# RoyiAvital/QuadraticProgramSolver

Measured on AMD Instinct MI355X. Metric: ADMM iterations/sec, higher is better.
Workload: dtype f64

## Files before the change

### quadraticprogramsolver_amd/csrc/k_loop.hip

```cpp
#include <cstdlib>

#include "qps_kernels.h"
#include "wave_reduce.h"
#include <hip/hip_ext.h>

namespace qps {

namespace {

template <typename T> __device__ __forceinline__ T wave_sum(T v) { return wave_sum_all(v); }
__device__ __forceinline__ unsigned long long absbits(double v) { return (unsigned long long)__double_as_longlong(fabs(v)); }
__device__ __forceinline__ unsigned long long wave_max_u64(unsigned long long v) {
#pragma unroll
    for (int o = 32; o > 0; o >>= 1) { unsigned long long t = __shfl_xor(v, o, 64); v = t > v ? t : v; }
    return v;
}

template <typename T, int RB, int TRI, int THREADS>
__global__ __launch_bounds__(THREADS) void k_gemv_rows(const T* __restrict__ S, int64_t ld, const T* __restrict__ v,
                                                   T* __restrict__ out, const T* __restrict__ out0, T alpha, T beta,
                                                   int r0, int c0, int c1, BatchStride bs) {
    using V = typename VecOf<T>::type;
    if (bs.active && !bs.active[blockIdx.y]) return;
    S += (int64_t)blockIdx.y * bs.mat; v += (int64_t)blockIdx.y * bs.vin; out += (int64_t)blockIdx.y * bs.vout;
// ... 30 lines not shown
            }
        }
    }
    __shared__ T red[THREADS / 64][RB];
#pragma unroll
    for (int i = 0; i < RB; ++i) acc[i] = wave_sum(acc[i]);
    if ((tid & 63) == 0) {
#pragma unroll
        for (int i = 0; i < RB; ++i) red[tid >> 6][i] = acc[i];
    }
    __syncthreads();
    if (tid < RB) {
        T s = T(0);
#pragma unroll
        for (int w = 0; w < THREADS / 64; ++w) s += red[w][tid];
        T r = alpha * s;
        if (beta != T(0)) r += beta * out0[rb + tid];
        out[rb + tid] = r;
    }
}

constexpr int GC_RT = 32;
template <typename T>
__global__ __launch_bounds__(256) void k_gemv_cols(const T* __restrict__ S, int64_t ld, const T* __restrict__ va,
                                                   const T* __restrict__ vb, T ca, T cb, T* __restrict__ part,
                                                   int64_t part_ld, int ncols) {
    using V = typename VecOf<T>::type;
    constexpr int VN = VecOf<T>::N;
    const int c = (blockIdx.x * 256 + threadIdx.x) * VN;
    if (c >= ncols) return;
    const int rt = blockIdx.y;
    const int rbase = rt * GC_RT;
    T acc[VN];
#pragma unroll
    for (int e = 0; e < VN; ++e) acc[e] = T(0);
    const T* Sp = S + (int64_t)rbase * ld + c;
#pragma unroll 8
    for (int i = 0; i < GC_RT; ++i) {
        T w = ca * va[rbase + i];
        if (vb) w += cb * vb[rbase + i];
        typedef T NV __attribute__((ext_vector_type(VN)));
        const NV a = __builtin_nontemporal_load(reinterpret_cast<const NV*>(Sp + (int64_t)i * ld));
#pragma unroll
        for (int e = 0; e < VN; ++e) acc[e] += a[e] * w;
    }
    V o;
    T* op = reinterpret_cast<T*>(&o);
#pragma unroll
    for (int e = 0; e < VN; ++e) op[e] = acc[e];
    *reinterpret_cast<V*>(part + (int64_t)rt * part_ld + c) = o;
}

template <typename T>
__global__ __launch_bounds__(256) void k_colsum(const T* __restrict__ part, int64_t part_ld, int ntiles,
                                                const T* __restrict__ a0, T s0, const T* __restrict__ a1, T s1,
                                                T* __restrict__ out, int ncols, BatchStride bs) {
    using V = typename VecOf<T>::type;
    constexpr int VN = VecOf<T>::N;
    if (bs.active && !bs.active[blockIdx.y]) return;
    part += (int64_t)blockIdx.y * bs.mat; out += (int64_t)blockIdx.y * bs.vout;
    if (a0) a0 += (int64_t)blockIdx.y * bs.vin;
    if (a1) a1 += (int64_t)blockIdx.y * bs.vin;
    constexpr int COLS = 128 / (int)sizeof(T);
    constexpr int CL = COLS / VN;
    constexpr int TL = 256 / CL;
    const int cl = threadIdx.x % CL, tl = threadIdx.x / CL;
    const int c = blockIdx.x * COLS + cl * VN;
    T acc[VN];
#pragma unroll
    for (int e = 0; e < VN; ++e) acc[e] = T(0);
    if (c < ncols) {
        int t = tl;
        for (; t + 7 * TL < ntiles; t += 8 * TL) {
            V v[8];
#pragma unroll
            for (int j = 0; j < 8; ++j) v[j] = *reinterpret_cast<const V*>(part + (int64_t)(t + TL * j) * part_ld + c);
#pragma unroll
            for (int j = 0; j < 8; ++j) {
                const T* vp = reinterpret_cast<const T*>(&v[j]);
#pragma unroll
                for (int e = 0; e < VN; ++e) acc[e] += vp[e];
            }
        }
        for (; t < ntiles; t += TL) {
            const V v = *reinterpret_cast<const V*>(part + (int64_t)t * part_ld + c);
            const T* vp = reinterpret_cast<const T*>(&v);
#pragma unroll
            for (int e = 0; e < VN; ++e) acc[e] += vp[e];
        }
    }
    __shared__ T red[TL][COLS + 1];
#pragma unroll
    for (int e = 0; e < VN; ++e) red[tl][cl * VN + e] = acc[e];
    __syncthreads();
    constexpr int PL = 256 / COLS;
    static_assert(TL % PL == 0 && (PL == 16 || PL == 8), "slab lanes per output");
    const int o = threadIdx.x / PL, pl = threadIdx.x % PL;
    T s = T(0);
#pragma unroll
    for (int k = 0; k < TL / PL; ++k) s += red[pl * (TL / PL) + k][o];
    s = (PL == 16) ? row16_sum_last(s) : oct_sum_all(s);
    const int oc = blockIdx.x * COLS + o;
    if (pl == PL - 1 && oc < ncols) {
        T r = s;
        if (a0) r += s0 * a0[oc];
        if (a1) r += s1 * a1[oc];
        out[oc] = r;
    }
}

template <typename T>
__global__ __launch_bounds__(256) void k_admm_update(int NP, int MP, const T* __restrict__ xx, const T* __restrict__ zz,
                                                     T* __restrict__ x, T* __restrict__ xp, T* __restrict__ z,
                                                     T* __restrict__ zp, T* __restrict__ y, const T* __restrict__ l,
                                                     const T* __restrict__ u, T alpha, T rho) {
    const int i = blockIdx.x * 256 + threadIdx.x;
    const T alpha1 = T(1) - alpha, rho1 = T(1) / rho;
    if (i < NP) {
        const T xo = x[i];
        xp[i] = xo;
        x[i] = alpha * xx[i] + alpha1 * xo;
    }
    if (i < MP) {
        const T zo = z[i], yo = y[i], zt = zz[i];
        zp[i] = zo;
        T t = alpha * zt + alpha1 * zo + rho1 * yo;
        const T lo = l[i], hi = u[i];
        const T zn = t > hi ? hi : (t < lo ? lo : t);
        z[i] = zn;
        y[i] = yo + rho * (alpha * zt + alpha1 * zo - zn);
    }
}

template <typename T>
__global__ __launch_bounds__(256) void k_check_norms(int n, int m, const T* __restrict__ Ax, const T* __restrict__ Px,
                                                     const T* __restrict__ Aty, const T* __restrict__ q,
                                                     const T* __restrict__ x, const T* __restrict__ xp,
                                                     const T* __restrict__ z, const T* __restrict__ zp,
                                                     unsigned long long* __restrict__ slots, int dual_only, BatchStride bs) {
    if (bs.active && !bs.active[blockIdx.y]) return;
    {
        const int64_t on = (int64_t)blockIdx.y * bs.vin, om = (int64_t)blockIdx.y * bs.vout;
        Ax += om; z += om; zp += om; Px += on; Aty += on; q += on; x += on; xp += on; slots += (int64_t)blockIdx.y * 16;
    }
    unsigned long long v[9];
#pragma unroll
    for (int k = 0; k < 9; ++k) v[k] = 0ull;
    for (int i = blockIdx.x * 256 + threadIdx.x; i < max(n, m); i += gridDim.x * 256) {
        if (i < m && !dual_only) {
            const double ax = (double)Ax[i], zi = (double)z[i];
            v[0] = max(v[0], absbits((double)(Ax[i] - z[i])));
            v[2] = max(v[2], absbits(ax));
            v[3] = max(v[3], absbits(zi));
            v[8] = max(v[8], absbits((double)(z[i] - zp[i])));
        }
        if (i < n) {
            v[1] = max(v[1], absbits((double)(Px[i] + q[i] + Aty[i])));
            v[4] = max(v[4], absbits((double)Px[i]));
            v[5] = max(v[5], absbits((double)Aty[i]));
            v[6] = max(v[6], absbits((double)q[i]));
            if (!dual_only) v[7] = max(v[7], absbits((double)(x[i] - xp[i])));
        }
    }
#pragma unroll
    for (int k = 0; k < 9; ++k) {
        v[k] = wave_max_u64(v[k]);
        if ((threadIdx.x & 63) == 0 && v[k] != 0ull) atomicMax(&slots[k], v[k]);
    }
}

__device__ __forceinline__ double jmax(double a, double b) { return (isnan(a) || isnan(b)) ? (double)NAN : (a > b ? a : b); }

__global__ void k_check_decide(const unsigned long long* __restrict__ slots, double* __restrict__ res, CheckScalars cs,
                               const double* __restrict__ rho_arr, const double* __restrict__ rhorho_arr,
                               const int* __restrict__ active) {
    if (threadIdx.x != 0) return;
    const int b = blockIdx.x;
    if (active && !active[b]) return;
    slots += (int64_t)b * 16; res += (int64_t)b * 8;
    if (rho_arr) { cs.rho = rho_arr[b]; cs.rhorho = rhorho_arr[b]; cs.convFlag = 1; }
    double nv[9];
    for (int k = 0; k < 9; ++k) nv[k] = __longlong_as_double((long long)slots[k]);
    const double MIN_VAL_RHO = 1e-3, MAX_VAL_RHO = 1e6;
    const double normResPrim = nv[0], normResDual = nv[1];
    const double maxNormPrim = jmax(nv[2], nv[3]);
    const double maxNormDual = jmax(jmax(nv[4], nv[5]), nv[6]);
    double rhorho = cs.rhorho;
    if (cs.adptRho) {
        const double numeratorVal = normResPrim * maxNormDual;
        const double denominatorVal = normResDual * maxNormPrim;
        const double t = cs.rho * sqrt(numeratorVal / denominatorVal);
        rhorho = t > MAX_VAL_RHO ? MAX_VAL_RHO : (t < MIN_VAL_RHO ? MIN_VAL_RHO : t);
    }
    const double epsPrim = cs.epsAbs + cs.epsRel * maxNormPrim;
    const double epsDual = cs.epsAbs + cs.epsRel * maxNormDual;
    int flag = cs.convFlag;
    if ((normResPrim < epsPrim) && (normResDual < epsDual)) flag = 3;
    if ((nv[7] <= cs.epsAdmm) && (nv[8] <= cs.epsAdmm)) flag = 2;
    res[0] = normResPrim; res[1] = normResDual; res[2] = maxNormPrim; res[3] = maxNormDual;
    res[4] = rhorho; res[5] = (double)flag; res[6] = nv[7]; res[7] = nv[8];
}

template <typename T> __global__ void k_fill(T* p, int64_t n, T v) {
    int64_t i = (int64_t)blockIdx.x * 256 + threadIdx.x;
    if (i < n) p[i] = v;
}
template <typename T> __global__ void k_convert(const double* __restrict__ s, T* __restrict__ d, int64_t n) {
    int64_t i = (int64_t)blockIdx.x * 256 + threadIdx.x;
    if (i < n) d[i] = (T)s[i];
}
template <typename T> __global__ void k_convert_back(const T* __restrict__ s, double* __restrict__ d, int64_t n) {
    int64_t i = (int64_t)blockIdx.x * 256 + threadIdx.x;
    if (i < n) d[i] = (double)s[i];
}

}

static int env_int(const char* name, int dflt) { const char* e = getenv(name); return e ? atoi(e) : dflt; }

template <typename T, int RB, int TH>
static void gemv_rows_launch(hipStream_t st, const T* S, int64_t ld, const T* v, T* out, const T* out0, T alpha, T beta, int r0,
                             int r1, int c0, int c1, int tri, BatchStride bs) {
    dim3 grid((r1 - r0 + RB - 1) / RB, bs.count);
#define QPS_GR(TRI) hipLaunchKernelGGL((k_gemv_rows<T, RB, TRI, TH>), grid, dim3(TH), 0, st, S, ld, v, out, out0, alpha, beta, r0, c0, c1, bs)
    if (tri == 0) QPS_GR(0); else if (tri == 1) QPS_GR(1); else QPS_GR(2);
#undef QPS_GR
}

template <typename T>
void gemv_rows(hipStream_t st, const T* S, int64_t ld, const T* v, T* out, const T* out0, T alpha, T beta, int r0, int r1,
               int c0, int c1, int tri, BatchStride bs) {
    if (r1 <= r0) return;
    static const int wide_th = env_int("QPS_GEMV_WIDE_THREADS", 512);
    static const int wide_rb = env_int("QPS_GEMV_WIDE_RB", 2);
    const bool wide = (c1 - c0) >= 4 * 256 * VecOf<T>::N;
    if (!wide) { gemv_rows_launch<T, 4, 256>(st, S, ld, v, out, out0, alpha, beta, r0, r1, c0, c1, tri, bs); return; }
#define QPS_W(RB, TH) gemv_rows_launch<T, RB, TH>(st, S, ld, v, out, out0, alpha, beta, r0, r1, c0, c1, tri, bs)
    if (wide_th == 512) { if (wide_rb == 4) QPS_W(4, 512); else QPS_W(VecOf<T>::N == 2 ? 2 : 4, 512); }
    else if (wide_th == 256) { if (wide_rb == 4) QPS_W(4, 256); else QPS_W(VecOf<T>::N == 2 ? 2 : 4, 256); }
    else { if (wide_rb == 4) QPS_W(4, 1024); else QPS_W(VecOf<T>::N == 2 ? 2 : 4, 1024); }
#undef QPS_W
}

int gemv_cols_tiles(int nrows) { return (nrows + GC_RT - 1) / GC_RT; }

template <typename T>
int gemv_cols_partial(hipStream_t st, const T* S, int64_t ld, const T* va, const T* vb, T ca, T cb, T* part,
                      int64_t part_ld, int nrows, int ncols) {
    constexpr int VN = VecOf<T>::N;
    const int tiles = gemv_cols_tiles(nrows);
    if (tiles == 0) return 0;
    dim3 grid((ncols + 256 * VN - 1) / (256 * VN), tiles), block(256);
    hipLaunchKernelGGL((k_gemv_cols<T>), grid, block, 0, st, S, ld, va, vb, ca, cb, part, part_ld, ncols);
    return tiles;
}

template <typename T>
void colsum(hipStream_t st, const T* part, int64_t part_ld, int ntiles, const T* a0, T s0, const T* a1, T s1, T* out,
            int ncols, BatchStride bs) {
    constexpr int cols_wg = 128 / (int)sizeof(T);
    if (g_launch_timing.start) {
        const LaunchTiming lt = g_launch_timing;
        g_launch_timing = LaunchTiming();
        hipExtLaunchKernelGGL((k_colsum<T>), dim3((ncols + cols_wg - 1) / cols_wg, bs.count), dim3(256), 0, st, lt.start, lt.stop, 0, part, part_ld, ntiles, a0, s0, a1, s1, out, ncols, bs);
        return;
    }
    hipLaunchKernelGGL((k_colsum<T>), dim3((ncols + cols_wg - 1) / cols_wg, bs.count), dim3(256), 0, st, part, part_ld, ntiles, a0, s0, a1, s1, out, ncols, bs);
}

template <typename T>
void admm_update(hipStream_t st, int NP, int MP, const T* xx, const T* zz, T* x, T* xp, T* z, T* zp, T* y, const T* l,
                 const T* u, T alpha, T rho) {
    const int N = NP > MP ? NP : MP;
    hipLaunchKernelGGL((k_admm_update<T>), dim3((N + 255) / 256), dim3(256), 0, st, NP, MP, xx, zz, x, xp, z, zp, y, l, u, alpha, rho);
}

template <typename T>
void check_convergence(hipStream_t st, int n, int m, const T* Ax, const T* Px, const T* Aty, const T* q, const T* x,
                       const T* xp, const T* z, const T* zp, unsigned long long* scratch, double* res_dev, CheckScalars cs,
                       int dual_only, BatchStride bs, const double* rho_arr, const double* rhorho_arr) {
    if (!dual_only) (void)hipMemsetAsync(scratch, 0, 16 * sizeof(unsigned long long) * bs.count, st);
    const int N = n > m ? n : m;
    int blocks = (N + 255) / 256;
    if (blocks > 1024) blocks = 1024;
    if (blocks < 1) blocks = 1;
    hipLaunchKernelGGL((k_check_norms<T>), dim3(blocks, bs.count), dim3(256), 0, st, n, m, Ax, Px, Aty, q, x, xp, z, zp, scratch, dual_only, bs);
    hipLaunchKernelGGL(k_check_decide, dim3(bs.count), dim3(64), 0, st, scratch, res_dev, cs, rho_arr, rhorho_arr, bs.active);
}

template <typename T> void fill(hipStream_t st, T* p, int64_t n, T v) {
    if (n <= 0) return;
    hipLaunchKernelGGL((k_fill<T>), dim3((unsigned)((n + 255) / 256)), dim3(256), 0, st, p, n, v);
}
template <typename T> void convert_copy(hipStream_t st, const double* src, T* dst, int64_t n) {
    if (n <= 0) return;
    hipLaunchKernelGGL((k_convert<T>), dim3((unsigned)((n + 255) / 256)), dim3(256), 0, st, src, dst, n);
}
template <typename T> void convert_back(hipStream_t st, const T* src, double* dst, int64_t n) {
    if (n <= 0) return;
    hipLaunchKernelGGL((k_convert_back<T>), dim3((unsigned)((n + 255) / 256)), dim3(256), 0, st, src, dst, n);
}

#define INST(T)                                                                                                              \
    template void gemv_rows<T>(hipStream_t, const T*, int64_t, const T*, T*, const T*, T, T, int, int, int, int, int, BatchStride); \
    template int gemv_cols_partial<T>(hipStream_t, const T*, int64_t, const T*, const T*, T, T, T*, int64_t, int, int);      \
    template void colsum<T>(hipStream_t, const T*, int64_t, int, const T*, T, const T*, T, T*, int, BatchStride);            \
    template void admm_update<T>(hipStream_t, int, int, const T*, const T*, T*, T*, T*, T*, T*, const T*, const T*, T, T);   \
    template void check_convergence<T>(hipStream_t, int, int, const T*, const T*, const T*, const T*, const T*, const T*,    \
                                       const T*, const T*, unsigned long long*, double*, CheckScalars, int, BatchStride,     \
                                       const double*, const double*);                                                        \
    template void fill<T>(hipStream_t, T*, int64_t, T);                                                                      \
    template void convert_copy<T>(hipStream_t, const double*, T*, int64_t);                                                  \
    template void convert_back<T>(hipStream_t, const T*, double*, int64_t);
INST(double)
INST(float)
#undef INST

}
```

### quadraticprogramsolver_amd/csrc/qps_dense.hip

```cpp
#include <memory>

#include "dense_chol.h"
#include "qps_batch.h"
#include "qps_internal.h"
#include "qps_kernels.h"
#include "qps_polish.h"

namespace qps {
namespace {

template <typename T> struct DenseSolver : SolverBase {
    int NP = 0, MP = 0;
    T *A = nullptr, *P = nullptr, *q = nullptr, *l = nullptr, *u = nullptr;
    T *PI = nullptr, *AA = nullptr, *M = nullptr, *S = nullptr, *tmp = nullptr, *dinv = nullptr; int* fail = nullptr;
    T *x = nullptr, *xp = nullptr, *z = nullptr, *zp = nullptr, *y = nullptr, *xx = nullptr, *zz = nullptr, *tt = nullptr, *yv = nullptr;
    T *part = nullptr, *part2 = nullptr, *sw_part = nullptr, *Ax = nullptr, *Px = nullptr, *Aty = nullptr;
    T* At = nullptr; void* small_out = nullptr; void* small_out_host = nullptr; bool small_ok = false;
    StreamLease lease; Arena arena;
    double* stage_mat = nullptr; int64_t stage_mat_count = 0;
    int pass_slabs = 0, pass_rpw = 0;
    unsigned long long* scratch = nullptr; double* res_dev = nullptr; double* res_host = nullptr; double* stage = nullptr;
    bool have_AA = false, factor_valid = false; double fac_rho = 0, fac_sigma = 0; int fac_nb = 0;
    int nb = 2048; int part_tiles = 0; int num_factorizations = 0;
    unsigned long long* pub = nullptr; unsigned* abort_dev = nullptr; unsigned sweep_epoch = 0; bool blocked_off = false, fac_premul = false;
    bool use_blocked() const { return !blocked_off && trsv_blocked_supported<T>(NP, nb); }
    struct IterGraph { int count; const void* xa; double rho, sigma, alpha; int nb; hipGraphExec_t exec; };
    std::vector<IterGraph> graphs;
    bool graphs_disabled = false;
    void drop_graphs() { for (auto& gr : graphs) (void)hipGraphExecDestroy(gr.exec); graphs.clear(); }
    hipGraphExec_t iter_graph(int count, T* xa, T* xb, double rho, double sigma, double alpha) {
        for (auto& gr : graphs) if (gr.count == count && gr.xa == xa && gr.rho == rho && gr.sigma == sigma && gr.alpha == alpha && gr.nb == nb) return gr.exec;
        if (graphs_disabled) return nullptr;
        if (graphs.size() >= 8) drop_graphs();
        hipGraph_t graph = nullptr; hipGraphExec_t exec = nullptr;
        if (hipStreamBeginCapture(st, hipStreamCaptureModeThreadLocal) != hipSuccess) { (void)hipGetLastError(); graphs_disabled = true; return nullptr; }
        for (int k = 0; k < count; ++k) {
            colsum<T>(st, part, NP, pass_slabs, xa, (T)sigma, q, T(-1), tt, NP);
            sweeps();
            apass<T>(st, false, A, NP, NP, MP, xx, xa, xb, z, y, l, u, (T)alpha, (T)rho, part, part2, NP, scratch);
            std::swap(xa, xb);
        }
        if (hipStreamEndCapture(st, &graph) != hipSuccess || graph == nullptr) { (void)hipGetLastError(); graphs_disabled = true; return nullptr; }
        const hipError_t e = hipGraphInstantiate(&exec, graph, nullptr, nullptr, 0);
        (void)hipGraphDestroy(graph);
        if (e != hipSuccess) { (void)hipGetLastError(); graphs_disabled = true; return nullptr; }
        graphs.push_back({count, xa, rho, sigma, alpha, nb, exec});
        return exec;
    }
    int prof_iter = 0;
    int sample_lvl(int slot) const { return (prof.level == 1 && prof_iter % 50 == slot) ? 1 : 2; }
    int cat_atw, cat_colsum, cat_fwd, cat_bwd, cat_ax, cat_upd, cat_chk, cat_pass, cat_passchk, cat_sweep, cat_xsum, cat_small;

    DenseSolver(int dev, int64_t n_, int64_t m_, int dt) {
        device = dev; n = n_; m = m_; dtype = dt;
        HIPC(hipSetDevice(device));
        NP = roundup(n, 64); MP = roundup(m, 64);
        const int64_t nn = (int64_t)NP * NP;
        part_tiles = gemv_cols_tiles(MP);
        pass_slabs = apass_plan<T>(NP, MP, &pass_rpw);
        const int slabs = std::max(std::max(part_tiles, pass_slabs), 1);
        small_ok = admm_small_supported<T>((int)n, (int)m, NP, MP);
        stage_mat_count = std::max((int64_t)n * n, (int64_t)m * n);
        if (stage_mat_count > ((int64_t)1 << 20)) stage_mat_count = 0;
        auto layout = [&](Arena& ar) {
            A = ar.take<T>((int64_t)MP * NP); P = ar.take<T>(nn); q = ar.take<T>(NP); l = ar.take<T>(MP); u = ar.take<T>(MP);
            PI = ar.take<T>(nn); AA = ar.take<T>(nn); M = ar.take<T>(nn); S = ar.take<T>(nn); tmp = ar.take<T>(nn);
            dinv = ar.take<T>((int64_t)(NP / 64) * 4096); fail = ar.take<int>(4);
            x = ar.take<T>(NP); xp = ar.take<T>(NP); xx = ar.take<T>(NP); tt = ar.take<T>(NP); yv = ar.take<T>(NP);
            z = ar.take<T>(MP); zp = ar.take<T>(MP); y = ar.take<T>(MP); zz = ar.take<T>(MP);
            part = ar.take<T>((int64_t)slabs * NP);
            part2 = ar.take<T>((int64_t)slabs * NP);
            sw_part = ar.take<T>((int64_t)std::max(sweep_fused_slabs<T>(NP), 1) * NP);
            Ax = ar.take<T>(MP); Px = ar.take<T>(NP); Aty = ar.take<T>(NP);
            scratch = ar.take<unsigned long long>(16); res_dev = ar.take<double>(16);
            pub = ar.take<unsigned long long>(trsv_blocked_pub_words<T>(NP));
            abort_dev = reinterpret_cast<unsigned*>(res_dev + 14);
            stage = ar.take<double>((int64_t)NP + 2 * (int64_t)MP + 64);
            if (small_ok) { At = ar.take<T>((int64_t)NP * MP); small_out = ar.take<double>(32); }
            if (stage_mat_count > 0) stage_mat = ar.take<double>(stage_mat_count);
        };
        layout(arena);
        st = prof.st = lease.acquire(device, arena.planned());
        HandleResources& res = lease.res;
        char* const recycled = res.block; res.block = nullptr;
        arena.commit(st, recycled, res.block_bytes);
        layout(arena);
        res_host = reinterpret_cast<double*>(res.pinned);
        small_out_host = small_ok ? reinterpret_cast<char*>(res.pinned) + 16 * sizeof(double) : nullptr;
        const double s = sizeof(T);
        cat_atw = prof.category("gemv_cols(A'w)", s * ((double)m * n + m + n));
        cat_colsum = prof.category("colsum(rhs)", s * ((double)part_tiles * n + 3.0 * n));
        cat_fwd = prof.category("trsv_forward", s * ((double)n * (n + 1) / 2 + 2.0 * n));
        cat_bwd = prof.category("trsv_backward", s * ((double)n * (n + 1) / 2 + 2.0 * n));
        cat_ax = prof.category("gemv_rows(Ax~)", s * ((double)m * n + m + n));
        cat_upd = prof.category("admm_update", s * (3.0 * n + 7.0 * m));
        cat_chk = prof.category("check_convergence", s * (2.0 * m * n + (double)n * n + 4.0 * n + 4.0 * m));
        cat_pass = prof.category("apass(fused A-pass)", s * ((double)m * n + 3.0 * n + 6.0 * m));
        cat_passchk = prof.category("apass(check variant)", s * ((double)m * n + 4.0 * n + 6.0 * m));
        cat_sweep = prof.category("sweeps(fused fwd+bwd, triangle read once)", s * ((double)n * (n + 1) / 2 + 2.0 * n + (double)sweep_fused_slabs<T>(NP) * n));
        cat_xsum = prof.category("colsum(x~ slabs)", s * ((double)sweep_fused_slabs<T>(NP) * n + n));
        cat_small = prof.category("admm_small(whole loop in one launch; bytes per iteration)", s * ((double)m * n + (double)n * n) + s * (6.0 * n + 10.0 * m));
    }
    ~DenseSolver() override {
        (void)hipSetDevice(device);
        (void)hipStreamSynchronize(st);
        trsv_blocked_forget_stream(device, st);
        drop_graphs();
        prof.release_events();
        lease.res.block = arena.base; lease.res.block_bytes = arena.bytes; arena.base = nullptr;
    }

    void upload_vec(const double* h, T* d, int64_t count) { HIPC(upload_staged<T>(st, stage, h, d, count)); }
    void download_vec(const T* d, double* h, int64_t count) { HIPC(download_staged<T>(st, stage, d, h, count)); }
    void upload_matrix(const double* h, int64_t ldh, int rows, int cols, T* d, int64_t ldd) {
        if (rows <= 0 || cols <= 0) return;
        if (stage_mat && (int64_t)rows * cols <= stage_mat_count) {
            HIPC(hipMemcpy2DAsync(stage_mat, sizeof(double) * (size_t)rows, h, sizeof(double) * (size_t)ldh, sizeof(double) * (size_t)rows, (size_t)cols, hipMemcpyHostToDevice, st));
            import_colmajor<T>(st, stage_mat, rows, rows, cols, d, ldd);
            HIPC(hipStreamSynchronize(st));
            return;
        }
        upload_matrix_panels<T>(st, device, h, ldh, rows, cols, d, ldd);
    }

    DenseChol<T> chol() const { return {st, (int)n, NP, MP, P, A, PI, AA, M, S, tmp, dinv, fail}; }
    void factorize(double rho, double sigma, bool rebuild_all) {
        const bool rebuild = rebuild_all || !have_AA;
        const DenseChol<T> c = chol();
        factor_valid = false;
        c.form(sigma, rho, rebuild, rebuild);
        have_AA = true;
        c.factor(nb, 1, use_blocked());
        char ctx[128]; snprintf(ctx, sizeof ctx, "rho=%g, sigma=%g; factorisation #%d of this handle", rho, sigma, ++num_factorizations);
        int f = 0;
        c.check("P + sigma I + rho A'A", ctx, &f);
        factor_valid = true; fac_rho = rho; fac_sigma = sigma; fac_nb = nb; fac_premul = use_blocked();
    }
    bool sweep_gave_up(bool fetched = false) {
        if (!fac_premul) return false;
        unsigned* h = reinterpret_cast<unsigned*>(res_host + 14);
// ... 13 lines not shown
            chol().sweeps(nb, tt, yv, xx, sw_part, BatchStride(), {&prof, cat_sweep, sample_lvl(13), cat_xsum, sample_lvl(21), cat_fwd, cat_bwd, 2});
            return;
        }
        if (sweep_epoch >= 0xfffffff0u) {
            HIPC(hipMemsetAsync(pub, 0, sizeof(unsigned long long) * (size_t)trsv_blocked_pub_words<T>(NP), st));
            sweep_epoch = 0;
        }
        TrsvBlockedPair gate(device, st);
        { ProfLaunchScope ps(prof, cat_fwd, sample_lvl(13)); trsv_blocked<T>(st, false, S, NP, NP, nb, tt, yv, pub, ++sweep_epoch, abort_dev); }
        { ProfLaunchScope ps(prof, cat_bwd, sample_lvl(21)); trsv_blocked<T>(st, true, S, NP, NP, nb, yv, xx, pub, ++sweep_epoch, abort_dev); }
    }
    void linear_solve(double rho, double sigma) {
        {
            ProfScope ps(prof, cat_atw, 1);
            gemv_cols_partial<T>(st, A, NP, z, y, (T)rho, T(-1), part, NP, MP, NP);
        }
        {
            ProfScope ps(prof, cat_colsum, 2);
            colsum<T>(st, part, NP, part_tiles, x, (T)sigma, q, T(-1), tt, NP);
        }
        sweeps();
        {
            ProfScope ps(prof, cat_ax, 2);
            gemv_rows<T>(st, A, NP, xx, zz, nullptr, T(1), T(0), 0, MP, 0, NP, 0);
        }
    }

    void solve(double* xh, const qps_params& p, qps_info* info) override {
        HIPC(hipSetDevice(device));
        blocked_off = false;
        int gave_up = 0; double t_lost = 0;
        const double t_begin = now_s();
        while (solve_once(xh, p, info)) {
            ++gave_up; t_lost = now_s() - t_begin;
            const int lvl = prof.level; prof.reset(); prof.level = lvl;
        }
        if (info) { info->sweepGaveUp = gave_up; info->cgExplicit = 0; info->tLoop += t_lost; }
    }
    bool solve_once(double* xh, const qps_params& p, qps_info* info) {
        if (p.linsys != QPS_LINSYS_AUTO && p.linsys != QPS_LINSYS_CHOLESKY)
            throw QpsError(QPS_ERR_UNSUPPORTED, "dense handles offer QPS_LINSYS_CHOLESKY only (qps_create_csc with dense_path = 0 for the CG and the sparse L D L' plugins)");
        const double t0 = now_s();
        nb = pick_nb<T>(p.trsvBlock, NP);
        double rho = p.rho, sigma = p.sigma; const double alpha = p.alpha;
        const double epsAdmm = std::fmin(p.epsAbs, p.epsRel) * 1e-2;
        int convFlag = QPS_CONV_NUM_ITR;
        const bool reuse = p.reuseFactor && factor_valid && fac_rho == rho && fac_sigma == sigma && fac_nb == nb && fac_premul == use_blocked();
        if (!reuse) factorize(rho, sigma, !p.reuseFactor || !have_AA || fac_sigma != sigma);
        upload_vec(xh, x, n);
        HIPC(hipMemsetAsync(xp, 0, sizeof(T) * NP, st));
        HIPC(hipMemsetAsync(z, 0, sizeof(T) * std::max(MP, 64), st));
        HIPC(hipMemsetAsync(y, 0, sizeof(T) * std::max(MP, 64), st));
        HIPC(hipMemsetAsync(zp, 0, sizeof(T) * std::max(MP, 64), st));
        HIPC(hipStreamSynchronize(st));
        const double t1 = now_s();
        double rhorho = rho;
        int ii = 0, nref = 0; double tref = 0, resP = NAN, resD = NAN;
        auto finish = [&](int iterations, double t_end, int variant) {
            PolishReport pr;
            if (p.polish) polish_dense<T>(st, n, m, NP, MP, P, A, q, l, u, y, x, part, p, &pr);
            download_vec(x, xh, n);
            if (info) {
                info->convFlag = convFlag; info->iterations = iterations; info->numRefactor = nref; info->cgIterations = 0;
                info->rhoFinal = rho; info->rhoProposed = rhorho; info->resPrim = resP; info->resDual = resD;
                info->tSetup = t1 - t0; info->tLoop = t_end - t1; info->tRefactor = tref;
                info->polishFlag = pr.flag; info->polishIterations = pr.minresIterations; info->tPolish = pr.seconds;
                info->trsvBlock = nb; info->sweepVariant = variant;
            }
            return false;
        };
        if (small_ok && p.loopVariant == 0 && (NP + nb - 1) / nb == 1) {
            transpose_small<T>(st, A, NP, MP, At);
            int it = 0;
            while (it < p.numIterations) {
                {
                    ProfScope ps(prof, cat_small, 1);
                    admm_small<T>(st, (int)n, (int)m, NP, MP, it, p.numIterations, p.numItrConv, p.adptRho, rho, rhorho, sigma, alpha, p.epsAbs,
                                  p.epsRel, epsAdmm, p.fctrRho, A, At, P, S, q, l, u, x, xp, z, y, small_out);
                }
                HIPC(hipMemcpyAsync(small_out_host, small_out, admm_small_out_bytes(), hipMemcpyDeviceToHost, st));
                HIPC(hipStreamSynchronize(st));
                prof.harvest();
                int last = 0, flag = 1, need = 0; double r8[8];
                admm_small_read(small_out_host, &last, &flag, &need, r8);
                it = last; convFlag = flag; rhorho = r8[4];
                if (!std::isnan(r8[0]) || !std::isnan(r8[1])) { resP = r8[0]; resD = r8[1]; }
                if (flag != QPS_CONV_NUM_ITR) break;
                if (need && it < p.numIterations) {
                    rho = rhorho; ++nref;
                    const double ta = now_s();
                    factorize(rho, sigma, false);
                    tref += now_s() - ta;
                }
            }
            return finish(it, now_s(), 4);
        }
        const bool fused = pass_slabs > 0 && p.loopVariant != 1;
        int rhs_slabs = 0;
        static const int graph_env = [] { const char* e = getenv("QPS_GRAPH"); return e ? atoi(e) : -1; }();
        const bool use_graph = fused && prof.level == 0 && p.numItrConv >= 3 && !fac_premul && (graph_env >= 0 ? graph_env != 0 : NP <= 2048);
        for (ii = 1; ii <= p.numIterations; ++ii) {
            bool changed = false;
            if (p.adptRho && ((rhorho * p.fctrRho < rho) || (rhorho > p.fctrRho * rho))) {
                rho = rhorho; ++nref; changed = true;
                const double ta = now_s();
                factorize(rho, sigma, false);
                tref += now_s() - ta;
            }
            const bool check = (ii % p.numItrConv == 0);
            if (use_graph && !changed && !check && rhs_slabs == pass_slabs) {
                int run = std::min(p.numItrConv - ii % p.numItrConv, p.numIterations - ii + 1) & ~1;
                hipGraphExec_t ge = run >= 2 ? iter_graph(run, x, xp, rho, sigma, alpha) : nullptr;
                if (ge) {
                    HIPC(hipGraphLaunch(ge, st));
                    ii += run - 1;
                    continue;
                }
            }
            if (!fused) {
                linear_solve(rho, sigma);
                {
                    ProfScope ps(prof, cat_upd, 2);
                    admm_update<T>(st, NP, MP, xx, zz, x, xp, z, zp, y, l, u, (T)alpha, (T)rho);
                }
                if (check) {
                    ProfScope ps(prof, cat_chk, 2);
                    gemv_rows<T>(st, A, NP, x, Ax, nullptr, T(1), T(0), 0, MP, 0, NP, 0);
                    gemv_rows<T>(st, P, NP, x, Px, nullptr, T(1), T(0), 0, NP, 0, NP, 0);
                    gemv_cols_partial<T>(st, A, NP, y, nullptr, T(1), T(0), part, NP, MP, NP);
                    colsum<T>(st, part, NP, part_tiles, nullptr, T(0), nullptr, T(0), Aty, NP);
                    CheckScalars cs{p.epsAbs, p.epsRel, epsAdmm, rho, rhorho, p.adptRho, convFlag};
                    check_convergence<T>(st, (int)n, (int)m, Ax, Px, Aty, q, x, xp, z, zp, scratch, res_dev, cs);
                }
            } else {
                if (changed && rhs_slabs > 0) {
                    ProfScope ps(prof, cat_atw, 2);
                    rhs_slabs = gemv_cols_partial<T>(st, A, NP, z, y, (T)rho, T(-1), part, NP, MP, NP);
                }
                prof_iter = ii;
                {
                    ProfLaunchScope ps(prof, cat_colsum, sample_lvl(29));
                    colsum<T>(st, part, NP, rhs_slabs, x, (T)sigma, q, T(-1), tt, NP);
                }
                sweeps();
                if (check) HIPC(hipMemsetAsync(scratch, 0, 16 * sizeof(unsigned long long), st));
                {
                    const int lvl = (prof.level == 1 && (check || ii % 50 != 38)) ? 3 : 1;
                    ProfLaunchScope ps(prof, check ? cat_passchk : cat_pass, lvl);
                    apass<T>(st, check, A, NP, NP, MP, xx, x, xp, z, y, l, u, (T)alpha, (T)rho, part, part2, NP, scratch);
                }
                std::swap(x, xp);
                rhs_slabs = pass_slabs;
                if (check) {
                    ProfScope ps(prof, cat_chk, 2);
                    colsum<T>(st, part2, NP, pass_slabs, nullptr, T(0), nullptr, T(0), Aty, NP);
                    gemv_rows<T>(st, P, NP, x, Px, nullptr, T(1), T(0), 0, NP, 0, NP, 0);
                    CheckScalars cs{p.epsAbs, p.epsRel, epsAdmm, rho, rhorho, p.adptRho, convFlag};
                    check_convergence<T>(st, (int)n, (int)m, Ax, Px, Aty, q, x, xp, z, zp, scratch, res_dev, cs, 1);
                }
            }
            if (check) {
                HIPC(hipMemcpyAsync(res_host, res_dev, 15 * sizeof(double), hipMemcpyDeviceToHost, st));
                HIPC(hipStreamSynchronize(st));
                prof.harvest();
                if (sweep_gave_up(true)) return true;
                resP = res_host[0]; resD = res_host[1]; rhorho = res_host[4]; convFlag = (int)res_host[5];
                if (convFlag != QPS_CONV_NUM_ITR) break;
            }
        }
        HIPC(hipStreamSynchronize(st));
        prof.harvest();
        if (sweep_gave_up()) return true;
        return finish(ii > p.numIterations ? p.numIterations : ii, now_s(), sweep_variant());
    }
    void polish(double* xh, const double* yh, const qps_params& p, qps_polish_report* rep) override {
        HIPC(hipSetDevice(device));
        upload_vec(xh, x, n); upload_vec(yh, y, m);
        PolishReport pr;
        polish_dense<T>(st, n, m, NP, MP, P, A, q, l, u, y, x, part, p, &pr);
        download_vec(x, xh, n);
        if (rep) {
            rep->flag = pr.flag; rep->refinements = pr.refinements; rep->minresIterations = pr.minresIterations;
            rep->numActiveLower = pr.numLower; rep->numActiveUpper = pr.numUpper; rep->reserved0 = 0; rep->relres = pr.relres; rep->seconds = pr.seconds;
        }
    }
    void get_dual(double* zh, double* yh) override {
        HIPC(hipSetDevice(device));
        if (zh) download_vec(z, zh, m);
        if (yh) download_vec(y, yh, m);
    }
    void linsys_init(double rho, double sigma, int linsys, int nbreq) override {
        HIPC(hipSetDevice(device));
        if (linsys != QPS_LINSYS_AUTO && linsys != QPS_LINSYS_CHOLESKY) throw QpsError(QPS_ERR_UNSUPPORTED, "dense handles support QPS_LINSYS_CHOLESKY only");
        nb = pick_nb<T>(nbreq, NP);
        blocked_off = false;
        factorize(rho, sigma, true);
    }
    void linsys_solve(const double* xh, const double* zh, const double* yh, double rho, double sigma, int changed,
                      double* xxh, double* zzh) override {
        HIPC(hipSetDevice(device));
        if (!factor_valid && !changed) throw QpsError(QPS_ERR_BAD_ARGUMENT, "qps_linsys_solve called before qps_linsys_init");
        if (changed) factorize(rho, sigma, false);
        upload_vec(xh, x, n); upload_vec(zh, z, m); upload_vec(yh, y, m);
        linear_solve(rho, sigma);
        if (sweep_gave_up()) { factorize(rho, sigma, false); linear_solve(rho, sigma); }
        download_vec(xx, xxh, n); download_vec(zz, zzh, m);
    }
    void operator_apply(int op, const double* in, double* out, double rho, double sigma) override {
        HIPC(hipSetDevice(device));
        auto Pin = [&](T* dst) { gemv_rows<T>(st, P, NP, xx, dst, nullptr, T(1), T(0), 0, NP, 0, NP, 0); };
        auto Ain = [&](T* dst) { if (m > 0) gemv_rows<T>(st, A, NP, xx, dst, nullptr, T(1), T(0), 0, MP, 0, NP, 0); };
        auto Atv = [&](const T* v, T* dst) {
            if (m > 0) { gemv_cols_partial<T>(st, A, NP, v, nullptr, T(1), T(0), part, NP, MP, NP); colsum<T>(st, part, NP, part_tiles, nullptr, T(0), nullptr, T(0), dst, NP); }
            else HIPC(hipMemsetAsync(dst, 0, sizeof(T) * NP, st));
        };
// ... 30 lines not shown
```

### quadraticprogramsolver_amd/csrc/qps_kernels.h

```cpp
#pragma once
#ifndef QPS_NT_SLABS
#define QPS_NT_SLABS 1
#endif
#include <hip/hip_runtime.h>
#include <stdint.h>

#include <atomic>
#include <thread>

namespace qps {

constexpr int kMaxDevices = 64;
int current_device();
int device_cu_count(int device);
struct PerDeviceOnce {
    std::atomic<unsigned char> state[kMaxDevices] = {};
    template <typename F> void once(int dev, F&& f) {
        if (dev < 0 || dev >= kMaxDevices) { f(); return; }
        if (state[dev].load(std::memory_order_acquire) == 2) return;
        unsigned char expect = 0;
        if (state[dev].compare_exchange_strong(expect, 1, std::memory_order_acq_rel)) { f(); state[dev].store(2, std::memory_order_release); return; }
        while (state[dev].load(std::memory_order_acquire) != 2) std::this_thread::yield();
    }
};

struct LaunchTiming { hipEvent_t start = nullptr, stop = nullptr; };
extern thread_local LaunchTiming g_launch_timing;


struct BatchStride { int count = 1; int64_t mat = 0, vin = 0, vout = 0; const int* active = nullptr; };

template <typename T> struct VecOf;
template <> struct VecOf<double> { using type = double2; static constexpr int N = 2; };
template <> struct VecOf<float>  { using type = float4;  static constexpr int N = 4; };

template <typename T>
void gemv_rows(hipStream_t st, const T* S, int64_t ld, const T* v, T* out, const T* out0, T alpha, T beta,
               int r0, int r1, int c0, int c1, int tri, BatchStride bs = BatchStride());

template <typename T>
int gemv_cols_partial(hipStream_t st, const T* S, int64_t ld, const T* va, const T* vb, T ca, T cb,
                      T* part, int64_t part_ld, int nrows, int ncols);
int gemv_cols_tiles(int nrows);

template <typename T>
void colsum(hipStream_t st, const T* part, int64_t part_ld, int ntiles, const T* a0, T s0, const T* a1, T s1,
            T* out, int ncols, BatchStride bs = BatchStride());

template <typename T>
void admm_update(hipStream_t st, int NP, int MP, const T* xx, const T* zz, T* x, T* xp, T* z, T* zp, T* y,
                 const T* l, const T* u, T alpha, T rho);

struct CheckScalars { double epsAbs, epsRel, epsAdmm, rho, rhorho; int adptRho; int convFlag; };
template <typename T>
void check_convergence(hipStream_t st, int n, int m, const T* Ax, const T* Px, const T* Aty, const T* q, const T* x,
                       const T* xp, const T* z, const T* zp, unsigned long long* scratch , double* res_dev,
                       CheckScalars cs, int dual_only = 0, BatchStride bs = BatchStride(), const double* rho_arr = nullptr,
                       const double* rhorho_arr = nullptr);

template <typename T> int apass_plan(int NP, int MP, int* rows_per_wg, int count = 1);
template <typename T> int apass_max_np();
struct PassBatch { int count = 1; int slabs = 0; const double* rho_arr = nullptr; const int* active = nullptr; int pq_me = 0; };
template <typename T>
void apass(hipStream_t st, bool check, const T* A, int64_t ld, int NP, int MP, const T* xx, const T* x_old, T* x_new, T* z,
           T* y, const T* l, const T* u, T alpha, T rho, T* part, T* part2, int64_t part_ld, unsigned long long* slots,
           PassBatch pb = PassBatch());
template <typename T> int apass_proxqp_slabs(int NP, int MP);
template <typename T>
int apass_kkt(hipStream_t st, const T* A, int64_t ld, int NP, int MP, const T* vx, const T* vlam, const T* mask, T delta, T* out_lam,
              T* part, int64_t part_ld);
template <typename T>
int apass_proxqp(hipStream_t st, const T* G, int64_t ld, int NP, int MP, int me, const T* x, T* x_scratch, T* slack, T* dual,
                 const T* g, T rho, T* part, int64_t part_ld);

template <typename T> bool sweep_fused_supported(int NP);
template <typename T> int sweep_fused_slabs(int NP, int count = 1);
template <typename T>
int sweep_fused(hipStream_t st, const T* S, int64_t ld, int NP, const T* v, T* part, int64_t part_ld, BatchStride bs = BatchStride());

template <typename T> struct PanelArgs {
    const T* Mat = nullptr; int64_t ld = 0; int rows = 0, K = 0;
    const T* B = nullptr; int npanel = 0;
    T* out = nullptr;
    const T* q = nullptr; T *x = nullptr, *xp = nullptr;
    T *z = nullptr, *zp = nullptr, *y = nullptr, *w = nullptr; const T *l = nullptr, *u = nullptr;
    const int* active = nullptr;
    T alpha = T(0), rho = T(1), sigma = T(0);
    const T *rho_row = nullptr, *rho1_row = nullptr;
};
enum class SharedPanelOp {
    product,
    rhs,
    forward,
    backward,
    backward_x,
    rows_zy,
    rows_zy_scaled,
    start_z
};
template <typename T> void shared_panel(hipStream_t st, SharedPanelOp op, const PanelArgs<T>& a);
bool shared_panel_small(int rows, int K, size_t elem);
template <typename T>
void shared_check(hipStream_t st, int n, int m, int NP, int MP, int npanel, const T* Ax, const T* Px, const T* Aty, const T* q, const T* x, const T* xp,
                  const T* z, const T* zp, unsigned long long* slots, double* res_dev, const int* active, double epsAbs, double epsRel, double epsAdmm,
                  double rho, const int* kd = nullptr, const int* ke = nullptr);
int shared_cert_blocks(int n, int m);
template <typename T>
void shared_deltas(hipStream_t st, int n, int m, int NP, int MP, int npanel, const T* x, const T* xp, const T* y, const T* yp, const T* l, const T* u,
                   const int* active, T* dx, T* dyh);
template <typename T>
void shared_certificates(hipStream_t st, int n, int m, int NP, int MP, int npanel, const T* dx, const T* dyh, const T* Adx, const T* Pdx, const T* Atdy,
// ... 118 lines not shown
```

### quadraticprogramsolver_amd/csrc/qps_runtime.hip

```cpp
#include <atomic>
#include <thread>

#include "qps_internal.h"
#include "qps_kernels.h"

namespace qps {
namespace {
constexpr size_t kRecycleBlockMax = (size_t)512 << 20;
constexpr int kRecyclePerDevice = 4;
std::mutex g_res_mu;
std::vector<HandleResources> g_res[kMaxDevices];
std::atomic<int> g_cus[kMaxDevices];
}
int current_device() { int dev = 0; if (hipGetDevice(&dev) != hipSuccess) { (void)hipGetLastError(); return 0; } return dev; }
int device_cu_count(int device) {
    if (device < 0 || device >= kMaxDevices) return 0;
    int c = g_cus[device].load(std::memory_order_acquire);
    if (c == 0) {
        if (hipDeviceGetAttribute(&c, hipDeviceAttributeMultiprocessorCount, device) != hipSuccess) { (void)hipGetLastError(); c = -1; }
        g_cus[device].store(c, std::memory_order_release);
    }
    return c > 0 ? c : 0;
}
HandleResources acquire_resources(int device, size_t block_need) {
    HandleResources r;
    {
        std::lock_guard<std::mutex> lk(g_res_mu);
        if (device >= 0 && device < kMaxDevices && !g_res[device].empty()) { r = g_res[device].back(); g_res[device].pop_back(); }
    }
    try {
        if (!r.st) HIPC(hipStreamCreateWithFlags(&r.st, hipStreamNonBlocking));
        if (!r.pinned) HIPC(hipHostMalloc(&r.pinned, kPinnedBytes));
    } catch (...) { recycle_resources(device, r); throw; }
    if (r.block && (r.block_bytes < block_need || r.block_bytes > 4 * block_need + ((size_t)1 << 20))) { (void)hipFree(r.block); r.block = nullptr; r.block_bytes = 0; }
    return r;
}
void recycle_resources(int device, HandleResources r) {
    if (r.block && r.block_bytes > kRecycleBlockMax) { (void)hipFree(r.block); r.block = nullptr; r.block_bytes = 0; }
    {
        std::lock_guard<std::mutex> lk(g_res_mu);
        if (device >= 0 && device < kMaxDevices && (int)g_res[device].size() < kRecyclePerDevice) { g_res[device].push_back(r); return; }
    }
    if (r.block) (void)hipFree(r.block);
    if (r.pinned) (void)hipHostFree(r.pinned);
    if (r.st) (void)hipStreamDestroy(r.st);
}
int host_threads() {
    static const int n = [] {
        const char* e = getenv("QPS_HOST_THREADS");
        const int hw = (int)std::max(1u, std::thread::hardware_concurrency());
        return std::max(1, std::min(e ? atoi(e) : 8, hw));
    }();
    return n;
}
namespace {
constexpr size_t kRingHalf = (size_t)32 << 20;
std::vector<PinnedRing> g_rings[kMaxDevices];
}
PinnedRing acquire_ring(int device) {
    PinnedRing r;
    {
        std::lock_guard<std::mutex> lk(g_res_mu);
        if (device >= 0 && device < kMaxDevices && !g_rings[device].empty()) { r = g_rings[device].back(); g_rings[device].pop_back(); }
    }
    if (!r.base) { HIPC(hipHostMalloc((void**)&r.base, 2 * kRingHalf)); r.half = kRingHalf; }
    return r;
}
void recycle_ring(int device, PinnedRing r) {
    if (!r.base) return;
    {
        std::lock_guard<std::mutex> lk(g_res_mu);
        if (device >= 0 && device < kMaxDevices && (int)g_rings[device].size() < kRecyclePerDevice) { g_rings[device].push_back(r); return; }
    }
    (void)hipHostFree(r.base);
}
thread_local LaunchTiming g_launch_timing;
ProfLaunchScope::ProfLaunchScope(Profiler& pr, int c, int lvl) : p(pr), cat(c), a(nullptr), b(nullptr), active(pr.on(lvl)) {
    if (active) { a = p.get(); b = p.get(); g_launch_timing.start = a; g_launch_timing.stop = b; }
}
ProfLaunchScope::~ProfLaunchScope() {
    if (!active) return;
    const bool consumed = (g_launch_timing.start == nullptr);
    g_launch_timing = LaunchTiming();
    if (consumed) p.pending.push_back({cat, a, b}); else { p.pool.push_back(a); p.pool.push_back(b); }
}
// ... 2 lines not shown
```

Baseline: 14570.

## Fuse Aty colsum, dual residual check and decision into one kernel

```diff
diff --git a/quadraticprogramsolver_amd/csrc/k_loop.hip b/quadraticprogramsolver_amd/csrc/k_loop.hip
--- a/quadraticprogramsolver_amd/csrc/k_loop.hip
+++ b/quadraticprogramsolver_amd/csrc/k_loop.hip
@@ -106,54 +106,62 @@
 }
 
 template <typename T>
+__device__ __forceinline__ T colsum_wg(const T* __restrict__ part, int64_t part_ld, int ntiles, int ncols, int bx) {
+    using V = typename VecOf<T>::type;
+    constexpr int VN = VecOf<T>::N;
+    constexpr int COLS = 128 / (int)sizeof(T);
+    constexpr int CL = COLS / VN;
+    constexpr int TL = 256 / CL;
+    const int cl = threadIdx.x % CL, tl = threadIdx.x / CL;
+    const int c = bx * COLS + cl * VN;
+    T acc[VN];
+#pragma unroll
+    for (int e = 0; e < VN; ++e) acc[e] = T(0);
+    if (c < ncols) {
+        int t = tl;
+        for (; t + 7 * TL < ntiles; t += 8 * TL) {
+            V v[8];
+#pragma unroll
+            for (int j = 0; j < 8; ++j) v[j] = *reinterpret_cast<const V*>(part + (int64_t)(t + TL * j) * part_ld + c);
+#pragma unroll
+            for (int j = 0; j < 8; ++j) {
+                const T* vp = reinterpret_cast<const T*>(&v[j]);
+#pragma unroll
+                for (int e = 0; e < VN; ++e) acc[e] += vp[e];
+            }
+        }
+        for (; t < ntiles; t += TL) {
+            const V v = *reinterpret_cast<const V*>(part + (int64_t)t * part_ld + c);
+            const T* vp = reinterpret_cast<const T*>(&v);
+#pragma unroll
+            for (int e = 0; e < VN; ++e) acc[e] += vp[e];
+        }
+    }
+    __shared__ T red[TL][COLS + 1];
+#pragma unroll
+    for (int e = 0; e < VN; ++e) red[tl][cl * VN + e] = acc[e];
+    __syncthreads();
+    constexpr int PL = 256 / COLS;
+    static_assert(TL % PL == 0 && (PL == 16 || PL == 8), "slab lanes per output");
+    const int o = threadIdx.x / PL, pl = threadIdx.x % PL;
+    T s = T(0);
+#pragma unroll
+    for (int k = 0; k < TL / PL; ++k) s += red[pl * (TL / PL) + k][o];
+    return (PL == 16) ? row16_sum_last(s) : oct_sum_all(s);
+}
+
+template <typename T>
 __global__ __launch_bounds__(256) void k_colsum(const T* __restrict__ part, int64_t part_ld, int ntiles,
                                                 const T* __restrict__ a0, T s0, const T* __restrict__ a1, T s1,
                                                 T* __restrict__ out, int ncols, BatchStride bs) {
-    using V = typename VecOf<T>::type;
-    constexpr int VN = VecOf<T>::N;
     if (bs.active && !bs.active[blockIdx.y]) return;
     part += (int64_t)blockIdx.y * bs.mat; out += (int64_t)blockIdx.y * bs.vout;
     if (a0) a0 += (int64_t)blockIdx.y * bs.vin;
     if (a1) a1 += (int64_t)blockIdx.y * bs.vin;
     constexpr int COLS = 128 / (int)sizeof(T);
-    constexpr int CL = COLS / VN;
-    constexpr int TL = 256 / CL;
-    const int cl = threadIdx.x % CL, tl = threadIdx.x / CL;
-    const int c = blockIdx.x * COLS + cl * VN;
-    T acc[VN];
-#pragma unroll
-    for (int e = 0; e < VN; ++e) acc[e] = T(0);
-    if (c < ncols) {
-        int t = tl;
-        for (; t + 7 * TL < ntiles; t += 8 * TL) {
-            V v[8];
-#pragma unroll
-            for (int j = 0; j < 8; ++j) v[j] = *reinterpret_cast<const V*>(part + (int64_t)(t + TL * j) * part_ld + c);
-#pragma unroll
-            for (int j = 0; j < 8; ++j) {
-                const T* vp = reinterpret_cast<const T*>(&v[j]);
-#pragma unroll
-                for (int e = 0; e < VN; ++e) acc[e] += vp[e];
-            }
-        }
-        for (; t < ntiles; t += TL) {
-            const V v = *reinterpret_cast<const V*>(part + (int64_t)t * part_ld + c);
-            const T* vp = reinterpret_cast<const T*>(&v);
-#pragma unroll
-            for (int e = 0; e < VN; ++e) acc[e] += vp[e];
-        }
-    }
-    __shared__ T red[TL][COLS + 1];
-#pragma unroll
-    for (int e = 0; e < VN; ++e) red[tl][cl * VN + e] = acc[e];
-    __syncthreads();
     constexpr int PL = 256 / COLS;
-    static_assert(TL % PL == 0 && (PL == 16 || PL == 8), "slab lanes per output");
+    const T s = colsum_wg<T>(part, part_ld, ntiles, ncols, blockIdx.x);
     const int o = threadIdx.x / PL, pl = threadIdx.x % PL;
-    T s = T(0);
-#pragma unroll
-    for (int k = 0; k < TL / PL; ++k) s += red[pl * (TL / PL) + k][o];
-    s = (PL == 16) ? row16_sum_last(s) : oct_sum_all(s);
     const int oc = blockIdx.x * COLS + o;
     if (pl == PL - 1 && oc < ncols) {
         T r = s;
@@ -225,6 +233,27 @@
 
 __device__ __forceinline__ double jmax(double a, double b) { return (isnan(a) || isnan(b)) ? (double)NAN : (a > b ? a : b); }
 
+__device__ __forceinline__ void check_decide(const double* nv, CheckScalars cs, double* res) {
+    const double MIN_VAL_RHO = 1e-3, MAX_VAL_RHO = 1e6;
+    const double normResPrim = nv[0], normResDual = nv[1];
+    const double maxNormPrim = jmax(nv[2], nv[3]);
+    const double maxNormDual = jmax(jmax(nv[4], nv[5]), nv[6]);
+    double rhorho = cs.rhorho;
+    if (cs.adptRho) {
+        const double numeratorVal = normResPrim * maxNormDual;
+        const double denominatorVal = normResDual * maxNormPrim;
+        const double t = cs.rho * sqrt(numeratorVal / denominatorVal);
+        rhorho = t > MAX_VAL_RHO ? MAX_VAL_RHO : (t < MIN_VAL_RHO ? MIN_VAL_RHO : t);
+    }
+    const double epsPrim = cs.epsAbs + cs.epsRel * maxNormPrim;
+    const double epsDual = cs.epsAbs + cs.epsRel * maxNormDual;
+    int flag = cs.convFlag;
+    if ((normResPrim < epsPrim) && (normResDual < epsDual)) flag = 3;
+    if ((nv[7] <= cs.epsAdmm) && (nv[8] <= cs.epsAdmm)) flag = 2;
+    res[0] = normResPrim; res[1] = normResDual; res[2] = maxNormPrim; res[3] = maxNormDual;
+    res[4] = rhorho; res[5] = (double)flag; res[6] = nv[7]; res[7] = nv[8];
+}
+
 __global__ void k_check_decide(const unsigned long long* __restrict__ slots, double* __restrict__ res, CheckScalars cs,
                                const double* __restrict__ rho_arr, const double* __restrict__ rhorho_arr,
                                const int* __restrict__ active) {
@@ -235,24 +264,80 @@
     if (rho_arr) { cs.rho = rho_arr[b]; cs.rhorho = rhorho_arr[b]; cs.convFlag = 1; }
     double nv[9];
     for (int k = 0; k < 9; ++k) nv[k] = __longlong_as_double((long long)slots[k]);
-    const double MIN_VAL_RHO = 1e-3, MAX_VAL_RHO = 1e6;
-    const double normResPrim = nv[0], normResDual = nv[1];
-    const double maxNormPrim = jmax(nv[2], nv[3]);
-    const double maxNormDual = jmax(jmax(nv[4], nv[5]), nv[6]);
-    double rhorho = cs.rhorho;
-    if (cs.adptRho) {
-        const double numeratorVal = normResPrim * maxNormDual;
-        const double denominatorVal = normResDual * maxNormPrim;
-        const double t = cs.rho * sqrt(numeratorVal / denominatorVal);
-        rhorho = t > MAX_VAL_RHO ? MAX_VAL_RHO : (t < MIN_VAL_RHO ? MIN_VAL_RHO : t);
-    }
-    const double epsPrim = cs.epsAbs + cs.epsRel * maxNormPrim;
-    const double epsDual = cs.epsAbs + cs.epsRel * maxNormDual;
-    int flag = cs.convFlag;
-    if ((normResPrim < epsPrim) && (normResDual < epsDual)) flag = 3;
-    if ((nv[7] <= cs.epsAdmm) && (nv[8] <= cs.epsAdmm)) flag = 2;
-    res[0] = normResPrim; res[1] = normResDual; res[2] = maxNormPrim; res[3] = maxNormDual;
-    res[4] = rhorho; res[5] = (double)flag; res[6] = nv[7]; res[7] = nv[8];
+    check_decide(nv, cs, res);
+}
+
+template <typename T>
+__global__ __launch_bounds__(256) void k_check_fused(int n, int ncols, const T* __restrict__ part2, int64_t part_ld, int ntiles,
+                                                     const T* __restrict__ Px, const T* __restrict__ q, T* __restrict__ Aty,
+                                                     unsigned long long* __restrict__ slots, unsigned long long* __restrict__ wg_max,
+                                                     double* __restrict__ res, const unsigned* __restrict__ abort_word, CheckScalars cs) {
+    constexpr int COLS = 128 / (int)sizeof(T);
+    constexpr int PL = 256 / COLS;
+    const int o = threadIdx.x / PL, pl = threadIdx.x % PL;
+    const int oc = blockIdx.x * COLS + o;
+    const bool mine = (pl == PL - 1) && oc < n;
+    T px = T(0), qq = T(0);
+    if (mine) { px = Px[oc]; qq = q[oc]; }
+    const T aty = colsum_wg<T>(part2, part_ld, ntiles, ncols, blockIdx.x);
+    if (pl == PL - 1 && oc < ncols) Aty[oc] = aty;
+    unsigned long long v1 = 0ull, v4 = 0ull, v5 = 0ull, v6 = 0ull;
+    if (mine) {
+        v1 = absbits((double)(px + qq + aty));
+        v4 = absbits((double)px); v5 = absbits((double)aty); v6 = absbits((double)qq);
+    }
+    v1 = wave_max_u64(v1); v4 = wave_max_u64(v4); v5 = wave_max_u64(v5); v6 = wave_max_u64(v6);
+    __shared__ unsigned long long s_w[4][4];
+    __shared__ unsigned long long s_slot[16];
+    __shared__ int s_last;
+    if ((threadIdx.x & 63) == 0) { unsigned long long* w = s_w[threadIdx.x >> 6]; w[0] = v1; w[1] = v4; w[2] = v5; w[3] = v6; }
+    __syncthreads();
+    if (threadIdx.x < 64) {
+        unsigned long long seen = 0ull;
+        if (threadIdx.x < 4) {
+            const int k = threadIdx.x;
+            unsigned long long mk = s_w[0][k];
+#pragma unroll
+            for (int w = 1; w < 4; ++w) mk = s_w[w][k] > mk ? s_w[w][k] : mk;
+            seen = atomicExch(&wg_max[4 * (int64_t)blockIdx.x + k], mk);
+        }
+        seen |= __shfl_xor(seen, 1, 64); seen |= __shfl_xor(seen, 2, 64);
+        if (threadIdx.x == 0) {
+            unsigned* ticket = reinterpret_cast<unsigned*>(slots + 15);
+            const unsigned t = __hip_atomic_fetch_add(ticket, 1u + (unsigned)(seen >> 63), __ATOMIC_RELAXED, __HIP_MEMORY_SCOPE_AGENT);
+            s_last = (t == gridDim.x - 1u);
+        }
+    }
+    __syncthreads();
+    if (!s_last) return;
+    unsigned long long r[4] = {0ull, 0ull, 0ull, 0ull};
+    for (int g = threadIdx.x; g < (int)gridDim.x; g += 256) {
+#pragma unroll
+        for (int k = 0; k < 4; ++k) { const unsigned long long t = atomicOr(&wg_max[4 * (int64_t)g + k], 0ull); r[k] = t > r[k] ? t : r[k]; }
+    }
+#pragma unroll
+    for (int k = 0; k < 4; ++k) r[k] = wave_max_u64(r[k]);
+    __syncthreads();
+    if ((threadIdx.x & 63) == 0) { unsigned long long* w = s_w[threadIdx.x >> 6]; w[0] = r[0]; w[1] = r[1]; w[2] = r[2]; w[3] = r[3]; }
+    if (threadIdx.x < 16) s_slot[threadIdx.x] = atomicExch(&slots[threadIdx.x], 0ull);
+    __syncthreads();
+    if (threadIdx.x != 0) return;
+    double nv[9];
+    for (int k = 0; k < 9; ++k) nv[k] = __longlong_as_double((long long)s_slot[k]);
+    {
+        const int slot_of[4] = {1, 4, 5, 6};
+#pragma unroll
+        for (int k = 0; k < 4; ++k) {
+            unsigned long long mk = s_w[0][k];
+#pragma unroll
+            for (int w = 1; w < 4; ++w) mk = s_w[w][k] > mk ? s_w[w][k] : mk;
+            nv[slot_of[k]] = __longlong_as_double((long long)mk);
+        }
+    }
+    double r8[8];
+    check_decide(nv, cs, r8);
+    for (int k = 0; k < 8; ++k) res[k] = r8[k];
+    reinterpret_cast<unsigned*>(res + 14)[0] = *abort_word;
 }
 
 template <typename T> __global__ void k_fill(T* p, int64_t n, T v) {
@@ -342,6 +427,17 @@
     hipLaunchKernelGGL(k_check_decide, dim3(bs.count), dim3(64), 0, st, scratch, res_dev, cs, rho_arr, rhorho_arr, bs.active);
 }
 
+template <typename T>
+int check_fused_wgs(int ncols) { return (ncols + 128 / (int)sizeof(T) - 1) / (128 / (int)sizeof(T)); }
+
+template <typename T>
+void check_fused(hipStream_t st, int n, int ncols, const T* part2, int64_t part_ld, int ntiles, const T* Px, const T* q, T* Aty,
+                 unsigned long long* scratch, unsigned long long* wg_max, double* res_mapped, const unsigned* abort_word, CheckScalars cs) {
+    constexpr int cols_wg = 128 / (int)sizeof(T);
+    hipLaunchKernelGGL((k_check_fused<T>), dim3((ncols + cols_wg - 1) / cols_wg), dim3(256), 0, st, n, ncols, part2, part_ld, ntiles, Px, q, Aty,
+                       scratch, wg_max, res_mapped, abort_word, cs);
+}
+
 template <typename T> void fill(hipStream_t st, T* p, int64_t n, T v) {
     if (n <= 0) return;
     hipLaunchKernelGGL((k_fill<T>), dim3((unsigned)((n + 255) / 256)), dim3(256), 0, st, p, n, v);
@@ -363,6 +459,9 @@
     template void check_convergence<T>(hipStream_t, int, int, const T*, const T*, const T*, const T*, const T*, const T*,    \
                                        const T*, const T*, unsigned long long*, double*, CheckScalars, int, BatchStride,     \
                                        const double*, const double*);                                                        \
+    template int check_fused_wgs<T>(int);                                                                                    \
+    template void check_fused<T>(hipStream_t, int, int, const T*, int64_t, int, const T*, const T*, T*, unsigned long long*,  \
+                                 unsigned long long*, double*, const unsigned*, CheckScalars);                                                    \
     template void fill<T>(hipStream_t, T*, int64_t, T);                                                                      \
     template void convert_copy<T>(hipStream_t, const double*, T*, int64_t);                                                  \
     template void convert_back<T>(hipStream_t, const T*, double*, int64_t);
diff --git a/quadraticprogramsolver_amd/csrc/qps_dense.hip b/quadraticprogramsolver_amd/csrc/qps_dense.hip
--- a/quadraticprogramsolver_amd/csrc/qps_dense.hip
+++ b/quadraticprogramsolver_amd/csrc/qps_dense.hip
@@ -20,6 +20,8 @@
     double* stage_mat = nullptr; int64_t stage_mat_count = 0;
     int pass_slabs = 0, pass_rpw = 0;
     unsigned long long* scratch = nullptr; double* res_dev = nullptr; double* res_host = nullptr; double* stage = nullptr;
+    unsigned long long* chk_wg = nullptr;
+    double* res_mapped = nullptr;
     bool have_AA = false, factor_valid = false; double fac_rho = 0, fac_sigma = 0; int fac_nb = 0;
     int nb = 2048; int part_tiles = 0; int num_factorizations = 0;
     unsigned long long* pub = nullptr; unsigned* abort_dev = nullptr; unsigned sweep_epoch = 0; bool blocked_off = false, fac_premul = false;
@@ -73,6 +75,7 @@
             sw_part = ar.take<T>((int64_t)std::max(sweep_fused_slabs<T>(NP), 1) * NP);
             Ax = ar.take<T>(MP); Px = ar.take<T>(NP); Aty = ar.take<T>(NP);
             scratch = ar.take<unsigned long long>(16); res_dev = ar.take<double>(16);
+            chk_wg = ar.take<unsigned long long>(4 * (int64_t)check_fused_wgs<T>(NP));
             pub = ar.take<unsigned long long>(trsv_blocked_pub_words<T>(NP));
             abort_dev = reinterpret_cast<unsigned*>(res_dev + 14);
             stage = ar.take<double>((int64_t)NP + 2 * (int64_t)MP + 64);
@@ -86,6 +89,7 @@
         arena.commit(st, recycled, res.block_bytes);
         layout(arena);
         res_host = reinterpret_cast<double*>(res.pinned);
+        { void* dp = nullptr; HIPC(hipHostGetDevicePointer(&dp, res.pinned, 0)); res_mapped = static_cast<double*>(dp); }
         small_out_host = small_ok ? reinterpret_cast<char*>(res.pinned) + 16 * sizeof(double) : nullptr;
         const double s = sizeof(T);
         cat_atw = prof.category("gemv_cols(A'w)", s * ((double)m * n + m + n));
@@ -205,6 +209,7 @@
         HIPC(hipMemsetAsync(z, 0, sizeof(T) * std::max(MP, 64), st));
         HIPC(hipMemsetAsync(y, 0, sizeof(T) * std::max(MP, 64), st));
         HIPC(hipMemsetAsync(zp, 0, sizeof(T) * std::max(MP, 64), st));
+        HIPC(hipMemsetAsync(scratch, 0, 16 * sizeof(unsigned long long), st));
         HIPC(hipStreamSynchronize(st));
         const double t1 = now_s();
         double rhorho = rho;
@@ -296,7 +301,6 @@
                     colsum<T>(st, part, NP, rhs_slabs, x, (T)sigma, q, T(-1), tt, NP);
                 }
                 sweeps();
-                if (check) HIPC(hipMemsetAsync(scratch, 0, 16 * sizeof(unsigned long long), st));
                 {
                     const int lvl = (prof.level == 1 && (check || ii % 50 != 38)) ? 3 : 1;
                     ProfLaunchScope ps(prof, check ? cat_passchk : cat_pass, lvl);
@@ -306,14 +310,13 @@
                 rhs_slabs = pass_slabs;
                 if (check) {
                     ProfScope ps(prof, cat_chk, 2);
-                    colsum<T>(st, part2, NP, pass_slabs, nullptr, T(0), nullptr, T(0), Aty, NP);
                     gemv_rows<T>(st, P, NP, x, Px, nullptr, T(1), T(0), 0, NP, 0, NP, 0);
                     CheckScalars cs{p.epsAbs, p.epsRel, epsAdmm, rho, rhorho, p.adptRho, convFlag};
-                    check_convergence<T>(st, (int)n, (int)m, Ax, Px, Aty, q, x, xp, z, zp, scratch, res_dev, cs, 1);
+                    check_fused<T>(st, (int)n, NP, part2, NP, pass_slabs, Px, q, Aty, scratch, chk_wg, res_mapped, abort_dev, cs);
                 }
             }
             if (check) {
-                HIPC(hipMemcpyAsync(res_host, res_dev, 15 * sizeof(double), hipMemcpyDeviceToHost, st));
+                if (!fused) HIPC(hipMemcpyAsync(res_host, res_dev, 15 * sizeof(double), hipMemcpyDeviceToHost, st));
                 HIPC(hipStreamSynchronize(st));
                 prof.harvest();
                 if (sweep_gave_up(true)) return true;
diff --git a/quadraticprogramsolver_amd/csrc/qps_kernels.h b/quadraticprogramsolver_amd/csrc/qps_kernels.h
--- a/quadraticprogramsolver_amd/csrc/qps_kernels.h
+++ b/quadraticprogramsolver_amd/csrc/qps_kernels.h
@@ -57,6 +57,10 @@
                        const T* xp, const T* z, const T* zp, unsigned long long* scratch , double* res_dev,
                        CheckScalars cs, int dual_only = 0, BatchStride bs = BatchStride(), const double* rho_arr = nullptr,
                        const double* rhorho_arr = nullptr);
+template <typename T>
+void check_fused(hipStream_t st, int n, int ncols, const T* part2, int64_t part_ld, int ntiles, const T* Px, const T* q, T* Aty,
+                 unsigned long long* scratch, unsigned long long* wg_max, double* res_mapped, const unsigned* abort_word, CheckScalars cs);
+template <typename T> int check_fused_wgs(int ncols);
 
 template <typename T> int apass_plan(int NP, int MP, int* rows_per_wg, int count = 1);
 template <typename T> int apass_max_np();
diff --git a/quadraticprogramsolver_amd/csrc/qps_runtime.hip b/quadraticprogramsolver_amd/csrc/qps_runtime.hip
--- a/quadraticprogramsolver_amd/csrc/qps_runtime.hip
+++ b/quadraticprogramsolver_amd/csrc/qps_runtime.hip
@@ -30,7 +30,7 @@
     }
     try {
         if (!r.st) HIPC(hipStreamCreateWithFlags(&r.st, hipStreamNonBlocking));
-        if (!r.pinned) HIPC(hipHostMalloc(&r.pinned, kPinnedBytes));
+        if (!r.pinned) HIPC(hipHostMalloc(&r.pinned, kPinnedBytes, hipHostMallocMapped | hipHostMallocCoherent));
     } catch (...) { recycle_resources(device, r); throw; }
     if (r.block && (r.block_bytes < block_need || r.block_bytes > 4 * block_need + ((size_t)1 << 20))) { (void)hipFree(r.block); r.block = nullptr; r.block_bytes = 0; }
     return r;
```

After: 14570. Within noise of the previous version (-0.0%).
